# davrempe/contact-human-dynamics

Hardware: NVIDIA H100
Metric: optimised frames/sec (batched phys-optim) (higher is better)
Workload: dtype f64

## Files before the change

### contact-human-dynamics_b200/csrc/chd_api.cu

```cuda
#include <cuda_runtime.h>

#include <cstdio>
#include <cstdlib>
#include <cstring>
#include <vector>

#include "../../include/chd.h"
#include "chd_dev.h"

__global__ void chd_k_stage_begin(ChdDev D);
__global__ void chd_k_eval(ChdDev D);
__global__ void chd_k_init(ChdDev D);
__global__ void chd_k_kkt(ChdDev D);
__global__ void chd_k_kkt_gwin(ChdDev D);
__global__ void chd_k_kcopy(ChdDev D);
__global__ void chd_k_curv(ChdDev D);
__global__ void chd_k_asm(ChdDev D);
__global__ void chd_k_fp64_peak(int mode, int iters, double* sink);
__global__ void chd_k_hess_base(ChdDev D);
__global__ void chd_k_hess_dur(ChdDev D);
__global__ void chd_k_hess_zero(ChdDev D);
__global__ void chd_k_hess_fin(ChdDev D, int mode);
__global__ void chd_k_tables(ChdDev D);
__global__ void chd_k_clear_dyn(ChdDev D);
// ... 363 lines not shown
  if (b->copy_stream) cudaStreamDestroy(b->copy_stream);
  if (b->stream) cudaStreamDestroy(b->stream);
  delete b;
}

int chd_phys_get_dims(const chd_phys_batch* b, chd_phys_dims* d) {
  if (!b || !d) return -1;
  const ChdHostBatch& hb = b->hb;
  d->batch = hb.B, d->n_max = hb.n_max, d->m_max = hb.m_max, d->slots_max = hb.slots_max, d->n_splines = hb.S;
  d->p_max = hb.Pmax, d->sets_max = hb.sets_max, d->na_max = hb.Na_max, d->nb_max = hb.nb_max, d->w_max = hb.w_max;
  d->frames_out_max = hb.fo_max;
  return 0;
}
int chd_phys_get_sizes(const chd_phys_batch* b, int32_t* s) {
  if (!b || !s) return -1;
  for (int i = 0; i < b->hb.B; ++i) {
    const ChdSeq& h = b->hb.seq[i];
    s[6 * i + 0] = h.n, s[6 * i + 1] = h.m, s[6 * i + 2] = h.nslots, s[6 * i + 3] = h.Na, s[6 * i + 4] = h.nb, s[6 * i + 5] = h.w;
  }
  return 0;
}
int chd_phys_get_sizes_fixed(const chd_phys_batch* b, int32_t* s) {
  if (!b || !s) return -1;
  for (int i = 0; i < b->hb.B; ++i) s[3 * i] = b->hb.seq[i].nb_fix, s[3 * i + 1] = b->hb.seq[i].w_fix, s[3 * i + 2] = b->hb.seq[i].n_dur;
  return 0;
}
int chd_phys_get_x(const chd_phys_batch* b, double* x) {
  if (!b || !x) return -1;
  if (b->host_only) {
    std::memcpy(x, b->hb.x0.data(), b->hb.x0.size() * sizeof(double));
    return 0;
  }
  CHD_CUDA(cudaStreamSynchronize(b->stream));
  CHD_CUDA(cudaMemcpy(x, b->D.x, (size_t)b->hb.B * b->hb.n_max * sizeof(double), cudaMemcpyDeviceToHost));
  return 0;
}
int chd_phys_set_x(chd_phys_batch* b, const double* x) {
  if (!b || !x || b->host_only) return -1;
  CHD_CUDA(cudaMemcpy(b->D.x, x, (size_t)b->hb.B * b->hb.n_max * sizeof(double), cudaMemcpyHostToDevice));
  chd_k_tables<<<b->hb.B, 64, 0, b->stream>>>(b->D);
  b->launches++;
  CHD_CUDA(cudaStreamSynchronize(b->stream));
  return 0;
}

int chd_phys_eval(chd_phys_batch* b, int32_t stage, double* cost, double* grad, double* g, double* jac_vals) {
  if (!b || stage < 0 || stage > 5 || b->host_only) return -1;
  const ChdHostBatch& hb = b->hb;
  int sched[1] = {stage};
  int rc = set_schedule(b, sched, 1, -1, 0);
  if (rc) return rc;
  {
    Timer t(b, KT_INIT);
    chd_k_stage_begin<<<hb.B, CHD_THREADS, 0, b->stream>>>(b->D);
  }
  launch_eval(b);
  CHD_CUDA(cudaStreamSynchronize(b->stream));
  CHD_CUDA(cudaGetLastError());
  const size_t B = hb.B;
  if (cost) {
    std::vector<double> c2(2 * B);
    CHD_CUDA(cudaMemcpy(c2.data(), b->D.cost, 2 * B * sizeof(double), cudaMemcpyDeviceToHost));
    for (size_t i = 0; i < B; ++i) cost[i] = c2[2 * i];
  }
  if (grad) CHD_CUDA(cudaMemcpy(grad, b->D.grad, B * hb.n_max * sizeof(double), cudaMemcpyDeviceToHost));
  if (g) CHD_CUDA(cudaMemcpy(g, b->D.g, B * hb.m_max * sizeof(double), cudaMemcpyDeviceToHost));
  if (jac_vals) CHD_CUDA(cudaMemcpy(jac_vals, b->D.Jv, B * hb.slots_max * sizeof(double), cudaMemcpyDeviceToHost));
  return 0;
}

int chd_phys_get_layout(const chd_phys_batch* b, int32_t* ent_ptr, int32_t* ent_col, double* row_lo, double* row_hi,
                        int32_t* row_set, int32_t* var_kkt, int32_t* row_kkt) {
  if (!b) return -1;
  const ChdHostBatch& hb = b->hb;
  if (ent_ptr) std::memcpy(ent_ptr, hb.ent_ptr.data(), hb.ent_ptr.size() * sizeof(int));
  if (ent_col) std::memcpy(ent_col, hb.ent_col.data(), hb.ent_col.size() * sizeof(int));
  if (row_lo) std::memcpy(row_lo, hb.row_lo.data(), hb.row_lo.size() * sizeof(double));
  if (row_hi) std::memcpy(row_hi, hb.row_hi.data(), hb.row_hi.size() * sizeof(double));
  if (row_set) std::memcpy(row_set, hb.row_set.data(), hb.row_set.size() * sizeof(int));
  if (var_kkt) std::memcpy(var_kkt, hb.var_kkt.data(), hb.var_kkt.size() * sizeof(int));
  if (row_kkt) std::memcpy(row_kkt, hb.row_kkt.data(), hb.row_kkt.size() * sizeof(int));
  return 0;
}

int chd_phys_get_slot_index(const chd_phys_batch* b, int32_t* ent_row, int32_t* col_ptr, int32_t* col_ent) {
  if (!b) return -1;
  const ChdHostBatch& hb = b->hb;
  if (ent_row) std::memcpy(ent_row, hb.ent_row.data(), hb.ent_row.size() * sizeof(int));
  if (col_ptr) std::memcpy(col_ptr, hb.col_ptr.data(), hb.col_ptr.size() * sizeof(int));
  if (col_ent) std::memcpy(col_ent, hb.col_ent.data(), hb.col_ent.size() * sizeof(int));
  return 0;
}

int chd_phys_get_ent_col(const chd_phys_batch* b, int32_t* ent_col) {
  if (!b || !ent_col) return -1;
  if (b->host_only) {
    std::memcpy(ent_col, b->hb.ent_col.data(), b->hb.ent_col.size() * sizeof(int));
    return 0;
  }
  CHD_CUDA(cudaStreamSynchronize(b->stream));
  CHD_CUDA(cudaMemcpy(ent_col, b->D.ent_col, b->hb.ent_col.size() * sizeof(int), cudaMemcpyDeviceToHost));
  return 0;
}

int chd_phys_get_duals(const chd_phys_batch* b, double* y, double* zL, double* zU, double* s, double* row_scale, double* obj_scale) {
  if (!b || b->host_only) return -1;
  const size_t B = b->hb.B, mm = B * b->hb.m_max;
  CHD_CUDA(cudaStreamSynchronize(b->stream));
  if (y) CHD_CUDA(cudaMemcpy(y, b->D.y, mm * sizeof(double), cudaMemcpyDeviceToHost));
  if (zL) CHD_CUDA(cudaMemcpy(zL, b->D.zL, mm * sizeof(double), cudaMemcpyDeviceToHost));
  if (zU) CHD_CUDA(cudaMemcpy(zU, b->D.zU, mm * sizeof(double), cudaMemcpyDeviceToHost));
  if (s) CHD_CUDA(cudaMemcpy(s, b->D.s, mm * sizeof(double), cudaMemcpyDeviceToHost));
  if (row_scale) CHD_CUDA(cudaMemcpy(row_scale, b->D.sc, mm * sizeof(double), cudaMemcpyDeviceToHost));
  if (obj_scale) {
    std::vector<ChdIpm> ipm(B);
    CHD_CUDA(cudaMemcpy(ipm.data(), b->D.ipm, B * sizeof(ChdIpm), cudaMemcpyDeviceToHost));
    for (size_t i = 0; i < B; ++i) obj_scale[i] = ipm[i].sf;
  }
  return 0;
}

int chd_phys_debug_ipm(const chd_phys_batch* b, int32_t i, double* out8) {
  if (!b || !out8 || b->host_only || !b->h_ipm || i < 0 || i >= b->hb.B) return -1;
  const ChdIpm& I = b->h_ipm[i];
  out8[0] = I.a_pr, out8[1] = I.a_du, out8[2] = I.dphi, out8[3] = I.phi0, out8[4] = I.theta0, out8[5] = I.theta_ref, out8[6] = I.mu, out8[7] = I.delta_w;
  for (int q = 0; q < 8; ++q) out8[8 + q] = I.dbg[q];
  return 0;
}

int chd_phys_stage_stats(const chd_phys_batch* b, double* stats) {
  if (!b || !stats || b->host_only || !b->h_ipm) return -1;
  const int B = b->hb.B;
  for (int s = 0; s < 6; ++s)
    for (int i = 0; i < B; ++i)
      for (int q = 0; q < 4; ++q) stats[((size_t)s * B + i) * 4 + q] = b->h_ipm[i].st_stat[s][q];
  return 0;
}

int chd_phys_solve_stage(chd_phys_batch* b, int32_t stage, int32_t max_iter, int32_t* status, int32_t* iters, double* stats) {
  if (!b || stage < 0 || stage > 5 || b->host_only) return -1;
  const int B = b->hb.B;
  int sched[1] = {stage};
  int rc = set_schedule(b, sched, 1, stage, max_iter);
  if (rc) return rc;
  if ((rc = run_schedule(b))) return rc;
  for (int i = 0; i < B; ++i) {
    const ChdIpm& I = b->h_ipm[i];
    if (status) status[i] = I.st_status[stage];
    if (iters) iters[i] = I.st_iters[stage];
    if (stats) {
      double* s = stats + 8 * i;
      s[0] = I.f, s[1] = I.E0, s[2] = I.viol_u, s[3] = I.dual_u, s[4] = I.compl_u, s[5] = I.mu, s[6] = I.delta_w, s[7] = I.ls_fail;
    }
    if (i == 0 && getenv("CHD_PROF")) fprintf(stderr, "chd prof (Mcycles) seq0 stage %d: err %.2f jasm %.2f hasm %.2f factor %.2f border %.2f back %.2f rec %.2f\n", stage, I.prof[0]/1e6, I.prof[1]/1e6, I.prof[2]/1e6, I.prof[3]/1e6, I.prof[4]/1e6, I.prof[5]/1e6, I.prof[6]/1e6);
  }
  return 0;
}

int chd_phys_sample_device(chd_phys_batch* b, double* out_device, void* stream) {
  if (!b || !out_device || b->host_only) return -1;
  cudaStream_t st = stream ? (cudaStream_t)stream : b->stream;
  if (st == b->stream) {
    Timer t(b, KT_SAMPLE);
    chd_k_sample<<<b->hb.B, 128, 0, st>>>(b->D, out_device, b->d_frames);
    return 0;
  }
  cudaEvent_t ev;
  CHD_CUDA(cudaEventCreateWithFlags(&ev, cudaEventDisableTiming));
  CHD_CUDA(cudaEventRecord(ev, b->stream));
  CHD_CUDA(cudaStreamWaitEvent(st, ev, 0));
  chd_k_sample<<<b->hb.B, 128, 0, st>>>(b->D, out_device, b->d_frames);
  CHD_CUDA(cudaEventRecord(ev, st));
  CHD_CUDA(cudaStreamWaitEvent(b->stream, ev, 0));
  CHD_CUDA(cudaEventDestroy(ev));
  return 0;
}

int chd_phys_sample(chd_phys_batch* b, double* out, int32_t* frames_out) {
  if (!b || !out || b->host_only) return -1;
  const ChdHostBatch& hb = b->hb;
  const size_t stride = 6 + 7 * (size_t)hb.n_ee_max, cnt = (size_t)hb.B * hb.fo_max * stride;
  CHD_CUDA(cudaMemsetAsync(b->d_samples, 0, cnt * sizeof(double), b->stream));
  int rc = chd_phys_sample_device(b, b->d_samples, nullptr);
  if (rc) return rc;
  CHD_CUDA(cudaMemcpyAsync(out, b->d_samples, cnt * sizeof(double), cudaMemcpyDeviceToHost, b->stream));
  if (frames_out) CHD_CUDA(cudaMemcpyAsync(frames_out, b->d_frames, hb.B * sizeof(int), cudaMemcpyDeviceToHost, b->stream));
  CHD_CUDA(cudaStreamSynchronize(b->stream));
  return 0;
}

int chd_phys_solve(chd_phys_batch* b, double* samples, int32_t* frames_out, int32_t* success, int32_t* stage_status,
                   int32_t* stage_iters) {
  if (!b || b->host_only) return -1;
  const ChdHostBatch& hb = b->hb;
  const int B = hb.B;
  const size_t stride = 6 + 7 * (size_t)hb.n_ee_max, snap = (size_t)B * hb.fo_max * stride;
  int sched[6] = {CHD_STAGE_11, CHD_STAGE_12, CHD_STAGE_21, CHD_STAGE_22, CHD_STAGE_3, CHD_STAGE_4};
  int rc = set_schedule(b, sched, 6, -1, 0);
  if (rc) return rc;
  if (samples) CHD_CUDA(cudaMemsetAsync(b->D.snapshots, 0, 3 * snap * sizeof(double), b->stream));
  if ((rc = run_schedule(b))) return rc;
  for (int i = 0; i < B; ++i) {
    const ChdIpm& I = b->h_ipm[i];
    if (success) success[2 * i] = I.st_status[CHD_STAGE_22] == 0, success[2 * i + 1] = I.st_status[CHD_STAGE_3] == 0 || I.st_status[CHD_STAGE_4] == 0;
    for (int s = 0; s < 6; ++s) {
      if (stage_status) stage_status[(size_t)s * B + i] = I.st_status[s];
      if (stage_iters) stage_iters[(size_t)s * B + i] = I.st_iters[s];
    }
  }
  if (samples) CHD_CUDA(cudaMemcpyAsync(samples, b->D.snapshots, 3 * snap * sizeof(double), cudaMemcpyDeviceToHost, b->stream));
  if (frames_out) CHD_CUDA(cudaMemcpyAsync(frames_out, b->d_frames, B * sizeof(int), cudaMemcpyDeviceToHost, b->stream));
  CHD_CUDA(cudaStreamSynchronize(b->stream));
  return 0;
}

int64_t chd_phys_launch_count(const chd_phys_batch* b) { return b ? b->launches : 0; }
int64_t chd_phys_h2d_bytes(const chd_phys_batch* b) { return b ? b->h2d_bytes : 0; }
int chd_phys_reset(chd_phys_batch* b) {
  if (!b || b->host_only) return -1;
  CHD_CUDA(cudaMemcpyAsync(b->D.x, b->d_x0, (size_t)b->hb.B * b->hb.n_max * sizeof(double), cudaMemcpyDeviceToDevice, b->stream));
  const ChdHostBatch& hb = b->hb;
  CHD_CUDA(cudaMemcpyAsync(b->D.poly_T, b->poly_T0, hb.poly_T.size() * sizeof(double), cudaMemcpyDeviceToDevice, b->stream));
  CHD_CUDA(cudaMemcpyAsync(b->D.poly_tend, b->poly_tend0, hb.poly_tend.size() * sizeof(double), cudaMemcpyDeviceToDevice, b->stream));
  CHD_CUDA(cudaMemcpyAsync(b->D.phase_tend, b->phase_tend0, hb.phase_tend.size() * sizeof(double), cudaMemcpyDeviceToDevice, b->stream));
  CHD_CUDA(cudaMemcpyAsync(b->D.ent_col, b->ent_col0, hb.ent_col.size() * sizeof(int), cudaMemcpyDeviceToDevice, b->stream));
  chd_k_clear_dyn<<<(hb.B + 127) / 128, 128, 0, b->stream>>>(b->D);
  b->launches++;
  return 0;
}
int chd_phys_set_timing(chd_phys_batch* b, int enable) {
  if (!b) return -1;
  b->timing = enable;
  return 0;
}
int chd_phys_kernel_times(chd_phys_batch* b, double* ms8, int64_t* launches8, int reset) {
  if (!b) return -1;
  for (int i = 0; i < KT_N; ++i) {
    if (ms8) ms8[i] = b->kt_ms[i];
    if (launches8) launches8[i] = b->kt_n[i];
    if (reset) b->kt_ms[i] = 0, b->kt_n[i] = 0;
  }
  return 0;
}

}
```

### contact-human-dynamics_b200/csrc/chd_dev.h

```cpp
#pragma once
#include "chd_core.h"
#include "chd_layout.h"

#define CHD_FILT_MAX 24
#define CHD_THREADS 512
#define CHD_KKT_THREADS 512
#define CHD_NL_GUARD 1.0
#define CHD_NL_FLOOR 1e-4
#define CHD_UNOBS_EPS 1e-14
#define CHD_DW_UNOBS 1e-4
#define CHD_CURV_MIN 1e-8

#define CHD_ROW_ACTIVE 1
#define CHD_ROW_EQ 2
#define CHD_ROW_HASL 4
#define CHD_ROW_HASU 8
#define CHD_ROW_WARM 16

#define CHD_PH_BEGIN 0
#define CHD_PH_RUN 1
#define CHD_PH_FINISHED 2
struct ChdIpm {
  int status;
  int iter, nfilt, ls_fail, max_iter, n_bounds, m_act, pad0;
  int stage, pos, phase, snap, step_ready;
  int last_p1;
  int warm;
  int dyn;
  int band_ovf;
  int kw_req;
  int st_status[6], st_iters[6];
  double mu, delta_w, sf, theta_max, theta_min, mu_filter, tau;
  double f, E0, viol_u, dual_u, compl_u;
  double phi0, theta0, dphi, a_pr, a_du;
  double dbg[8];
  double dw_floor;
  int af_cnt, af_off;
  int af_it, af_pad;
  double af_E;
  double theta_ref;
  double filt[2 * CHD_FILT_MAX];
  double st_stat[6][4];
  double prof[8];
};

struct ChdStageDev {
  unsigned set_mask;
  int max_iter;
  int snap_after;
  int opt_dur;
  double w_data[3], w_vel[3], w_acc[3], w_dur;
};

struct ChdDev {
  int B, S, Pmax, n_max, m_max, slots_max, sets_max, tab_max, F_max, Kd_max, Kr_max, Na_max, nb_max, w_max, par_stride,
      n_ee_max, fo_max, Ph_max, win_smem, nbc_max, Q, Qfix, nbt, win_tiles, pan_doubles;
  size_t kstride;
  const ChdSeq* seq;
  double *poly_T, *poly_tend;
  const double *node_const, *par, *t_dyn, *t_rom, *t_data, *row_lo, *row_hi, *dur0;
  const int *node_var, *itab, *ent_ptr, *var_kkt, *row_kkt, *row_set, *poly_ph;
  int* ent_col;
  double *poly_Tt, *poly_tendt;
  double* jty;
  const int *ent_row, *col_ptr, *col_ent;
  const ChdSet* sets;
  double* phase_tend;
  double *x, *xt, *dx, *grad;
  double *g, *gt;
  double* Jv;
  int* rflag;
  unsigned char* unobs;
  double *sc, *dL, *dU, *s, *y, *zL, *zU, *ds, *dy, *dzL, *dzU;
  double* cost;
  double* Kwork;
  double* Kbase;
  double* sol;
  double* scratch;
  double *rhs0, *rhs1;
  size_t scratch_stride;
  ChdIpm* ipm;
  const ChdStageDev* stages;
  int sched[8], nsched;
  double* snapshots;
};

#define CHD_TOL 1e-3
#define CHD_CONSTR_VIOL_TOL 1e-4
#define CHD_DUAL_INF_TOL 1.0
#define CHD_COMPL_INF_TOL 1e-4
#define CHD_MU_INIT 0.1
#define CHD_KAPPA_EPS 10.0
#define CHD_KAPPA_MU 0.2
#define CHD_THETA_MU 1.5
#define CHD_TAU_MIN 0.99
#define CHD_KAPPA1 1e-2
#define CHD_KAPPA2 1e-2
#define CHD_KAPPA_SIGMA 1e10
#define CHD_S_MAX 100.0
#define CHD_SCAL_MAX_GRAD 100.0
#define CHD_BOUND_RELAX 1e-8
#define CHD_DELTA_W0 1e-4
#define CHD_DELTA_C 1e-8
#define CHD_DW_POLISH 1.0
#define CHD_DW_MIN 1e-8
#define CHD_AF_N 10
#define CHD_AF_MIN 1e-10
#define CHD_DW_MAX 1e4
#define CHD_DW_INC 4.0
#define CHD_DW_DEC 3.0
#define CHD_MAX_BACKTRACK 25
#define CHD_GAMMA_THETA 1e-5
#define CHD_GAMMA_PHI 1e-5
#define CHD_S_PHI 2.3
#define CHD_S_THETA 1.1
#define CHD_ETA_PHI 1e-8
#define CHD_INF 1e19

#if defined(__CUDACC__) || defined(CHD_HOST_EMU)
__device__ __forceinline__ void chd_stage_advance(const ChdDev& D, ChdIpm& I, int status, int snap_after) {
  I.st_status[I.stage] = status;
  I.st_iters[I.stage] = I.iter;
  I.st_stat[I.stage][0] = I.f, I.st_stat[I.stage][1] = I.E0, I.st_stat[I.stage][2] = I.viol_u, I.st_stat[I.stage][3] = I.dual_u;
  I.last_p1 = I.stage + 1;
  I.step_ready = 0;
  I.kw_req = 0;
  I.pos += 1;
  if (I.stage == CHD_STAGE_3 && status == 0 && I.pos < D.nsched && D.sched[I.pos] == CHD_STAGE_4) I.pos += 1;
  else if (I.stage == CHD_STAGE_3 && status != 0 && I.pos < D.nsched && D.sched[I.pos] == CHD_STAGE_4) snap_after = -1;
  I.snap = snap_after;
  if (I.pos < D.nsched) I.stage = D.sched[I.pos], I.phase = CHD_PH_BEGIN;
  else I.phase = CHD_PH_FINISHED;
}
#endif
```

### contact-human-dynamics_b200/csrc/chd_kernels.cu

```cuda
#include <cuda_runtime.h>

#include "chd_block.cuh"
#include "chd_eval.cuh"

__global__ void chd_k_stage_begin(ChdDev D) {
  const int b = blockIdx.x;
  if (D.ipm[b].phase != CHD_PH_BEGIN) return;
  const ChdStageDev sg = D.stages[D.ipm[b].stage];
  const int max_iter = sg.max_iter;
  const ChdSeq* h = D.seq + b;
  if (sg.opt_dur && h->n_dur == 0) {
    __syncthreads();
    if (threadIdx.x == 0) {
      D.ipm[b].iter = 0;
      chd_stage_advance(D, D.ipm[b], -3, sg.snap_after);
    }
    return;
  }
  const bool warm = sg.opt_dur && D.ipm[b].last_p1 == CHD_STAGE_22 + 1;
  int* rf = D.rflag + (size_t)b * D.m_max;
  const double* lo = D.row_lo + (size_t)b * D.m_max;
  const double* hi = D.row_hi + (size_t)b * D.m_max;
  const int* rset = D.row_set + (size_t)b * D.m_max;
  for (int r = threadIdx.x; r < D.m_max; r += blockDim.x) {
    int f = 0;
    if (r < h->m && (sg.set_mask & CHD_MASK(rset[r]))) {
      f = CHD_ROW_ACTIVE;
      if (lo[r] == hi[r]) f |= CHD_ROW_EQ;
      else {
        if (lo[r] > -CHD_INF) f |= CHD_ROW_HASL;
        if (hi[r] < CHD_INF) f |= CHD_ROW_HASU;
      }
      if (warm && (rf[r] & CHD_ROW_ACTIVE)) f |= CHD_ROW_WARM;
    }
    rf[r] = f;
    D.g[(size_t)b * D.m_max + r] = 0.0;
  }
  if (sg.opt_dur) {
    ChdCtx c;
    chd_make_ctx(D, b, D.x + (size_t)b * D.n_max, c);
    chd_tables_from_x(c, c.x, D.poly_T + (size_t)b * D.S * D.Pmax, D.poly_tend + (size_t)b * D.S * D.Pmax,
                      D.phase_tend + (size_t)b * D.n_ee_max * D.Ph_max);
  }
  if (threadIdx.x == 0) {
    ChdIpm& I = D.ipm[b];
    I.status = 1;
    I.iter = 0;
    I.nfilt = 0;
    I.ls_fail = 0;
    I.max_iter = max_iter;
    I.warm = warm;
    if (sg.opt_dur) I.dyn = 1;
    I.band_ovf = 0;
    if (!warm) I.mu = CHD_MU_INIT, I.sf = 1.0, I.delta_w = CHD_DELTA_W0;
    else I.delta_w = fmax(I.delta_w, CHD_DELTA_W0);
    I.mu_filter = -1.0;
    I.dw_floor = CHD_DW_MIN, I.af_cnt = 0, I.af_off = 0, I.af_it = 0, I.af_E = 0.0;
    for (int q = 0; q < 8; ++q) I.prof[q] = 0.0;
    for (int q = 40; q < 48; ++q) I.filt[q] = 0.0;
  }
}

__global__ void __launch_bounds__(CHD_THREADS) chd_k_eval(ChdDev D) {
  extern __shared__ double sm[];
  const int b = blockIdx.x;
  if (D.ipm[b].phase != CHD_PH_BEGIN && D.ipm[b].phase != CHD_PH_RUN) return;
  const ChdStageDev sg = D.stages[D.ipm[b].stage];
  const ChdSeq* h = D.seq + b;
  double* xs = sm;
  double* gs = sm + D.n_max;
  double* red = sm + 2 * D.n_max;
  const double* x = D.x + (size_t)b * D.n_max;
  for (int i = threadIdx.x; i < h->n; i += blockDim.x) xs[i] = x[i], gs[i] = 0.0;
  __syncthreads();
  ChdCtx c;
  chd_make_ctx(D, b, xs, c);
  c.dyn = D.ipm[b].dyn;
  c.opt_dur = sg.opt_dur;
  chd_eval_all<true>(c, sg, D.g + (size_t)b * D.m_max, D.Jv + (size_t)b * D.slots_max, gs, D.cost + 2 * b, red);
  double* grad = D.grad + (size_t)b * D.n_max;
  for (int i = threadIdx.x; i < h->n; i += blockDim.x) grad[i] = gs[i];
}

__global__ void __launch_bounds__(CHD_THREADS) chd_k_init(ChdDev D) {
  __shared__ double red[CHD_THREADS];
  const int b = blockIdx.x;
  if (D.ipm[b].phase != CHD_PH_BEGIN) return;
  const ChdSeq* h = D.seq + b;
  const size_t ro = (size_t)b * D.m_max;
  const int* vk = D.var_kkt + (size_t)b * D.n_max;
  const double* grad = D.grad + (size_t)b * D.n_max;
  double gm = 0.0;
  for (int i = threadIdx.x; i < h->n; i += blockDim.x)
    if (vk[i] >= 0) gm = fmax(gm, fabs(grad[i]));
  gm = chd_block_max(gm, red);
  const bool warm = D.ipm[b].warm;
  const double mu0 = D.ipm[b].mu;
  const double sf = warm ? D.ipm[b].sf : (gm > CHD_SCAL_MAX_GRAD ? CHD_SCAL_MAX_GRAD / gm : 1.0);
  const int* ep = D.ent_ptr + (size_t)b * (D.m_max + 1);
  const int* ec = D.ent_col + (size_t)b * D.slots_max;
  const double* Jv = D.Jv + (size_t)b * D.slots_max;
  int nb_l = 0;
  for (int r = threadIdx.x; r < h->m; r += blockDim.x) {
    const int f = D.rflag[ro + r];
    if (!(f & CHD_ROW_ACTIVE)) continue;
    if (f & CHD_ROW_WARM) {
      if (!(f & CHD_ROW_EQ)) nb_l += ((f & CHD_ROW_HASL) ? 1 : 0) + ((f & CHD_ROW_HASU) ? 1 : 0);
      continue;
    }
    double rm = 0.0;
    for (int e = ep[r]; e < ep[r + 1]; ++e) {
      const int col = ec[e];
      if (col >= 0 && vk[col] >= 0) rm = fmax(rm, fabs(Jv[e]));
    }
    double sc = rm > CHD_SCAL_MAX_GRAD ? CHD_SCAL_MAX_GRAD / rm : 1.0;
    sc = fmax(sc, 1e-8);
    D.sc[ro + r] = sc;
    const double lo = D.row_lo[ro + r] * sc, hi = D.row_hi[ro + r] * sc;
    const double d = sc * D.g[ro + r];
    D.y[ro + r] = 0.0;
    if (f & CHD_ROW_EQ) {
      D.dL[ro + r] = lo, D.dU[ro + r] = hi, D.s[ro + r] = d, D.zL[ro + r] = 0.0, D.zU[ro + r] = 0.0;
      continue;
    }
    const bool hl = f & CHD_ROW_HASL, hu = f & CHD_ROW_HASU;
    const double dL = hl ? lo - CHD_BOUND_RELAX * fmax(1.0, fabs(lo)) : -INFINITY;
    const double dU = hu ? hi + CHD_BOUND_RELAX * fmax(1.0, fabs(hi)) : INFINITY;
    double s = d;
    if (hl) {
      double pL = CHD_KAPPA1 * fmax(1.0, fabs(dL));
      if (hu) pL = fmin(pL, CHD_KAPPA2 * (dU - dL));
      s = fmax(s, dL + pL);
    }
    if (hu) {
      double pU = CHD_KAPPA1 * fmax(1.0, fabs(dU));
      if (hl) pU = fmin(pU, CHD_KAPPA2 * (dU - dL));
      s = fmin(s, dU - pU);
    }
    D.dL[ro + r] = dL, D.dU[ro + r] = dU, D.s[ro + r] = s;
    D.zL[ro + r] = hl ? (warm ? mu0 / (s - dL) : 1.0) : 0.0;
    D.zU[ro + r] = hu ? (warm ? mu0 / (dU - s) : 1.0) : 0.0;
    nb_l += (hl ? 1 : 0) + (hu ? 1 : 0);
  }
  const double nbnd = chd_block_sum((double)nb_l, red);
  int act = 0;
  for (int r = threadIdx.x; r < h->m; r += blockDim.x) act += (D.rflag[ro + r] & CHD_ROW_ACTIVE) ? 1 : 0;
  const double nact = chd_block_sum((double)act, red);
  if (threadIdx.x == 0) {
    D.ipm[b].sf = sf;
    D.ipm[b].n_bounds = (int)nbnd;
    D.ipm[b].m_act = (int)nact;
  }
}

__global__ void __launch_bounds__(CHD_THREADS) chd_k_linesearch(ChdDev D) {
  extern __shared__ double sm[];
  __shared__ int s_ok, s_ftype, s_trust;
  __shared__ double s_cost;
  const int b = blockIdx.x;
  ChdIpm& I = D.ipm[b];
  if (I.phase != CHD_PH_RUN || !I.step_ready) return;
  const ChdStageDev sg = D.stages[I.stage];
  const ChdSeq* h = D.seq + b;
  const int n = h->n, m = h->m, tid = threadIdx.x, nt = blockDim.x;
  const size_t ro = (size_t)b * D.m_max, vo = (size_t)b * D.n_max;
  const int* rf = D.rflag + ro;
  double* xt = sm;
  double* red = sm + D.n_max;
  const double* x = D.x + vo;
  const double* dx = D.dx + vo;
  double* gt = D.gt + ro;
  const double mu = I.mu, sf = I.sf, theta = I.theta0, phi0 = I.phi0, dphi = I.dphi, a_pr = I.a_pr, a_du = I.a_du;
  if (a_pr == 0.0 && dphi == 0.0) {
    if (tid == 0) I.iter += 1, I.step_ready = 0;
    return;
  }
  ChdCtx c;
  chd_make_ctx(D, b, xt, c);
  c.dyn = I.dyn;
  c.opt_dur = sg.opt_dur;
  if (sg.opt_dur) {
    c.poly_T = D.poly_Tt + (size_t)b * D.S * D.Pmax;
    c.poly_tend = D.poly_tendt + (size_t)b * D.S * D.Pmax;
    const size_t cnt = (size_t)D.S * D.Pmax;
    for (size_t i = tid; i < cnt; i += nt) {
      D.poly_Tt[(size_t)b * cnt + i] = D.poly_T[(size_t)b * cnt + i];
      D.poly_tendt[(size_t)b * cnt + i] = D.poly_tend[(size_t)b * cnt + i];
    }
    __syncthreads();
  }
  const double theta_ref = I.theta_ref;
  double alpha = a_pr;
  int ls = 0;
  bool accepted = false, ftype = false;
  for (ls = 0; ls < CHD_MAX_BACKTRACK; ++ls) {
    for (int i = tid; i < n; i += nt) xt[i] = x[i] + alpha * dx[i];
    __syncthreads();
    if (sg.opt_dur) {
      if (tid == 0) s_trust = 0;
      __syncthreads();
      if (tid < h->n_ee) {
        double t = 0.0, t0 = 0.0;
        int bad = 0;
        for (int k = 0; k < h->n_phases[tid] - 1; ++k) {
          t += xt[h->dur_xoff[tid] + k];
          t0 += c.dur0[(size_t)tid * c.Ph_max + k];
          if (fabs(t - t0) > CHD_TAU_TRUST) bad = 1;
        }
        if (bad) s_trust = 1;
      }
      chd_tables_from_x(c, xt, D.poly_Tt + (size_t)b * D.S * D.Pmax, D.poly_tendt + (size_t)b * D.S * D.Pmax, nullptr);
// ... 186 lines not shown
```

### contact-human-dynamics_b200/csrc/chd_kkt.cu

```cuda
#include <cuda_runtime.h>

#include "chd_block.cuh"
#include "chd_eval.cuh"
#include "chd_kkt_tiles.cuh"

__device__ __forceinline__ void chd_hess_sample(const ChdCtx& c, const ChdKT& K, const int* vk, int s, const ChdSpl* P, const double* sign, int np,
                                                int deriv, double wgt, int lane, double* ws) {
  const bool tau = c.opt_dur && s >= 2 && deriv == 0;
  if (lane < 28) {
    const int pa = lane / 14, q = lane % 14;
    double v0 = 0.0, v1 = 0.0, v2 = 0.0;
    int ia = -1;
    if (pa < np) {
      if (q < 12) {
        const int va = P[pa].var[q];
        const double wa = sign[pa] * chd_slot_w(P[pa], deriv, q);
        if (va >= 0 && wa != 0.0) {
          ia = vk[va];
          v0 = q % 3 == 0 ? wa : 0.0, v1 = q % 3 == 1 ? wa : 0.0, v2 = q % 3 == 2 ? wa : 0.0;
        }
      } else if (tau) {
        ChdTau u;
        chd_spl_tau(c, s, s - 2, P[pa], u);
        const int var = q == 12 ? u.va : u.vb;
// ... 515 lines not shown
  int na;
  {
    const int g1 = lane + 32;
    const bool act0 = lane < Gm && (lane >= GB || lane < tq) && gnz[lane];
    const bool act1 = g1 < Gm && (g1 >= GB || g1 < tq) && gnz[g1 < 96 ? g1 : 0];
    const unsigned m0 = __ballot_sync(0xffffffffu, act0), m1 = __ballot_sync(0xffffffffu, act1);
    const unsigned below = (1u << lane) - 1u;
    const int n0 = __popc(m0);
    na = n0 + __popc(m1);
    if (act0) cmp[__popc(m0 & below)] = (unsigned char)lane;
    if (act1) cmp[n0 + __popc(m1 & below)] = (unsigned char)g1;
    __syncwarp();
  }
  auto corner = [&](const double* X, const double* Y, int bi, int bj) {
    double* Cc = c.cc + (size_t)(bi * 8 + (lane >> 2)) * nbp8 + bj * 8 + 2 * (lane & 3);
    double c0 = Cc[0], c1 = Cc[1];
    chd_tile_mma(c0, c1, X, Y, lane);
    Cc[0] = c0, Cc[1] = c1;
  };
  const int step = c.nwarp - 1, r8 = (lane >> 2) * 8 + 2 * (lane & 3);
  const int nb2 = (na + 1) >> 1, nblk = nb2 * (nb2 + 1) / 2;
  for (int p = warp - 1; p < nblk; p += step) {
    const int bi = s_pairs[p] >> 8, bj = s_pairs[p] & 255;
    const int i1 = 2 * bi + 1, j1 = 2 * bj + 1;
    const bool vi1 = i1 < na, vj1 = j1 < na;
    int gi[2], gj[2];
    gi[0] = cmp[2 * bi], gi[1] = cmp[i1 & 63];
    gj[0] = cmp[2 * bj], gj[1] = cmp[j1 & 63];
    double2 xf[2], yf[2];
    xf[0] = *reinterpret_cast<const double2*>(xpan + gi[0] * 64 + 2 * lane);
    yf[0] = *reinterpret_cast<const double2*>(ypan + gj[0] * 64 + 2 * lane);
    xf[1] = vi1 ? *reinterpret_cast<const double2*>(xpan + gi[1] * 64 + 2 * lane) : make_double2(0.0, 0.0);
    yf[1] = vj1 ? *reinterpret_cast<const double2*>(ypan + gj[1] * 64 + 2 * lane) : make_double2(0.0, 0.0);
    double* Cp[4];
    double2 cv[4];
#pragma unroll
    for (int t = 0; t < 4; ++t) {
      const int a = t & 1, cl = t >> 1;
      bool ok = (a == 0 || vi1) && (cl == 0 || vj1) && !(bi == bj && a == 0 && cl == 1);
      const int g_i = gi[a], g_j = gj[cl];
      ok = ok && !(g_i == 0 && g_j == 0);
      Cp[t] = nullptr;
      if (ok) {
        if (g_i < GB) Cp[t] = band_tile(g_i, g_j);
        else if (g_j < GB) Cp[t] = bord_tile(g_i - GB, g_j);
        else corner(xpan + g_i * 64, ypan + g_j * 64, g_i - GB, g_j - GB);
      }
      if (Cp[t]) cv[t] = *reinterpret_cast<const double2*>(Cp[t] + r8);
    }
#pragma unroll
    for (int t = 0; t < 4; ++t)
      if (Cp[t]) {
        const double2 xa = xf[t & 1], yb = yf[t >> 1];
        asm volatile("mma.sync.aligned.m8n8k4.row.col.f64.f64.f64.f64 {%0,%1}, {%2}, {%3}, {%0,%1};"
                     : "+d"(cv[t].x), "+d"(cv[t].y)
                     : "d"(-xa.x), "d"(yb.x));
      }
#pragma unroll
    for (int t = 0; t < 4; ++t)
      if (Cp[t]) {
        const double2 xa = xf[t & 1], yb = yf[t >> 1];
        asm volatile("mma.sync.aligned.m8n8k4.row.col.f64.f64.f64.f64 {%0,%1}, {%2}, {%3}, {%0,%1};"
                     : "+d"(cv[t].x), "+d"(cv[t].y)
                     : "d"(-xa.y), "d"(yb.y));
        *reinterpret_cast<double2*>(Cp[t] + r8) = cv[t];
      }
  }
}

template <class BandTile, class BordTile>
__device__ __forceinline__ void chd_kkt_update_wide(const ChdKktCtx& c, const unsigned short* s_pairs, const int* gnz, int GB, int npairs,
                                                    int tq, const BandTile& band_tile, const BordTile& bord_tile) {
  const int lane = c.lane, nwarp = c.nwarp, nbp8 = c.nbp8;
  const double *xpan = c.xpan, *ypan = c.ypan;
  double* cc = c.cc;
  const int r8 = (lane >> 2) * 8 + 2 * (lane & 3);
  int p = c.warp - 1;
  while (p < npairs) {
    struct { double* C; const double *X, *Y; } tl[4];
    int nq = 0;
    while (nq < 4 && p < npairs) {
      const int gi = s_pairs[p] >> 8, gj = s_pairs[p] & 255;
      p += nwarp - 1;
      if ((gi < GB && gi >= tq) || (gj < GB && gj >= tq) || !gnz[gi] || !gnz[gj]) continue;
      if (gi == 0 && gj == 0) continue;
      const double* X = xpan + gi * 64;
      const double* Y = ypan + gj * 64;
      if (gi < GB) {
        tl[nq].C = band_tile(gi, gj), tl[nq].X = X, tl[nq].Y = Y, ++nq;
      } else if (gj < GB) {
        tl[nq].C = bord_tile(gi - GB, gj), tl[nq].X = X, tl[nq].Y = Y, ++nq;
      } else {
        const int bi = gi - GB, bj = gj - GB;
        for (int e = lane; e < 64; e += 32) {
          const int r = e >> 3, cq = e & 7;
          double acc = 0.0;
#pragma unroll
          for (int kk = 0; kk < 8; ++kk) acc += X[r * 8 + kk] * Y[cq * 8 + kk];
          cc[(bi * 8 + r) * nbp8 + bj * 8 + cq] -= acc;
        }
      }
    }
    double c0[4], c1[4];
#pragma unroll
    for (int i = 0; i < 4; ++i)
      if (i < nq) c0[i] = tl[i].C[r8], c1[i] = tl[i].C[r8 + 1];
#pragma unroll
    for (int i = 0; i < 4; ++i)
      if (i < nq) {
        chd_tile_mma(c0[i], c1[i], tl[i].X, tl[i].Y, lane);
        tl[i].C[r8] = c0[i], tl[i].C[r8 + 1] = c1[i];
      }
  }
}

template <bool WS>
__device__ __forceinline__ void chd_kkt_factor(const ChdKktCtx& c, int& s_fail) {
  const ChdKT& K = c.K;
  const int tid = c.tid, nt = c.nt, lane = c.lane, warp = c.warp, nwarp = c.nwarp;
  const int Qs = c.Qs, Q = c.Q, nbt = c.nbt, nbp8 = c.nbp8, nbc = c.nbc, nbt_s = c.nbt_s;
  double *cc = c.cc, *ypan = c.ypan, *xpan = c.xpan, *dinv = c.dinv, *win = c.win, *bwin = c.bwin;
  for (int i = tid; i < nbp8 * nbp8; i += nt) cc[i] = K.corn[i];
  if (WS) {
    for (int idx = tid; idx < Q * Q * 64; idx += nt) {
      const int e = idx & 63, pr = idx >> 6, J = pr / Q, t = pr % Q;
      if (J + t < Q && J < nbc && J + t < nbc) win[chd_win_slot(J + t, J, Q) * 64 + e] = K.band[((size_t)J * Qs + t) * 64 + e];
    }
    for (int idx = tid; idx < Q * nbt * 64; idx += nt) {
      const int J = idx / (nbt * 64);
      if (J < nbc) bwin[idx] = K.bord[(size_t)J * nbt * 64 + idx % (nbt * 64)];
    }
  }
  __syncthreads();
  __shared__ int s_rs[2][96];
  __shared__ int s_gnz[2][96];
  __shared__ unsigned short s_pairs[3000];
  __shared__ unsigned char s_cmp[CHD_KKT_THREADS / 32][64];
  __shared__ __align__(16) double s_winv[2][64];
  const int GB = K.q, Gm = K.q + nbt_s, npairs = Gm * (Gm + 1) / 2;
  for (int p = tid; p < npairs && p < 3000; p += nt) {
    int gi = (int)((sqrt(8.0 * p + 1.0) - 1.0) * 0.5);
    while (gi * (gi + 1) / 2 > p) --gi;
    while ((gi + 1) * (gi + 2) / 2 <= p) ++gi;
    s_pairs[p] = (unsigned short)((gi << 8) | (p - gi * (gi + 1) / 2));
  }
  auto tri = [](int a_, int b_) { return a_ > b_ ? a_ * (a_ + 1) / 2 + b_ : b_ * (b_ + 1) / 2 + a_; };
  for (int g = tid; g < GB; g += nt) s_rs[0][g] = (1 + g) % Q;
  for (int g = tid; g < 96; g += nt) s_gnz[0][g] = 0, s_gnz[1][g] = 0;
  if (warp == 0) {
    const bool ok = chd_tile_ldl(WS ? win : K.band, dinv, s_winv[0], lane);
    if (!ok && lane == 0) s_fail = 1;
  }
  __syncthreads();
  int kslot = 0, cur = 0;
  for (int Kc = 0; Kc < nbc; ++Kc, cur ^= 1) {
    const int tq = min(K.q, nbc - 1 - Kc);
    const int* rs = s_rs[cur];
    auto band_tile = [&](int gi, int gj) -> double* {
      return WS ? win + (size_t)tri(rs[gi], rs[gj]) * 64 : K.band + ((size_t)(Kc + 1 + gj) * Qs + (gi - gj)) * 64;
    };
    auto bord_tile = [&](int bi, int gj) -> double* {
      return WS ? bwin + ((size_t)rs[gj] * nbt + bi) * 64 : K.bord + ((size_t)(Kc + 1 + gj) * nbt + bi) * 64;
    };
    double* Tkk = WS ? win + (size_t)tri(kslot, kslot) * 64 : K.band + (size_t)Kc * Qs * 64;
    double* Bk = WS ? bwin + (size_t)kslot * nbt * 64 : K.bord + (size_t)Kc * nbt * 64;
    const double* dv = dinv + 8 * cur;
    {
      const double* wv = s_winv[cur];
      const int r = lane >> 2, k = lane & 3;
      const double2 wf = *reinterpret_cast<const double2*>(wv + 2 * lane);
      const double d0 = dv[2 * k], d1 = dv[2 * k + 1];
      const int f0 = r * 8 + chd_frag_col(2 * k), f1 = r * 8 + chd_frag_col(2 * k + 1);
      for (int g = warp; g < tq + nbt_s; g += nwarp) {
        const bool band_t = g < tq;
        const int pg = band_t ? g : GB + (g - tq);
        const double* A = band_t ? (WS ? win + (size_t)tri(rs[g], kslot) * 64 : K.band + ((size_t)Kc * Qs + 1 + g) * 64) : Bk + (g - tq) * 64;
        const double ax = A[r * 8 + k], ay = A[r * 8 + k + 4];
        double c0 = 0.0, c1 = 0.0;
        asm volatile("mma.sync.aligned.m8n8k4.row.col.f64.f64.f64.f64 {%0,%1}, {%2}, {%3}, {%0,%1};"
                     : "+d"(c0), "+d"(c1)
                     : "d"(ax), "d"(wf.x));
        asm volatile("mma.sync.aligned.m8n8k4.row.col.f64.f64.f64.f64 {%0,%1}, {%2}, {%3}, {%0,%1};"
                     : "+d"(c0), "+d"(c1)
                     : "d"(ay), "d"(wf.y));
        const double x0 = c0 * d0, x1 = c1 * d1;
        ypan[pg * 64 + f0] = c0, ypan[pg * 64 + f1] = c1;
        xpan[pg * 64 + f0] = x0, xpan[pg * 64 + f1] = x1;
        double* G = band_t ? K.band + ((size_t)Kc * Qs + 1 + g) * 64 : K.bord + ((size_t)Kc * nbt + (g - tq)) * 64;
        *reinterpret_cast<double2*>(G + r * 8 + 2 * k) = make_double2(x0, x1);
        const bool nz = __any_sync(0xffffffffu, x0 != 0.0 || x1 != 0.0);
        if (lane == 0 && nz) s_gnz[cur][pg] = 1;
      }
    }
    if (WS)
      for (int e = tid; e < 64; e += nt) K.band[(size_t)Kc * Qs * 64 + e] = Tkk[e];
    __syncthreads();
    const int In = Kc + Q;
    if (WS && In < nbc) {
      for (int idx = tid - 32; idx < Q * 32 + nbt_s * 32; idx += nt - 32) {
        if (idx < 0) break;
        const int tile = idx >> 5, off = (idx & 31) * 2;
        if (tile < Q) {
          const int J = tile < GB ? Kc + 1 + tile : In;
          double* dst = tile < GB ? win + (size_t)tri(kslot, rs[tile]) * 64 : Tkk;
          chd_copy16(dst + off, K.band + ((size_t)J * Qs + (In - J)) * 64 + off, WS);
        } else {
          chd_copy16(Bk + (tile - Q) * 64 + off, K.bord + (size_t)In * nbt * 64 + (tile - Q) * 64 + off, WS);
        }
      }
    }
    if (warp == 0) {
      if (tq >= 1) {
        double* Tn = band_tile(0, 0);
        chd_tile_sub_xyT(Tn, xpan, ypan, lane);
        __syncwarp();
        const bool ok = chd_tile_ldl(Tn, dinv + 8 * (cur ^ 1), s_winv[cur ^ 1], lane);
        if (!ok && lane == 0) s_fail = 1;
      }
    } else {
      if (warp == 1) {
        for (int g = lane; g < GB; g += 32) {
          int v = kslot + 2 + g;
          while (v >= Q) v -= Q;
          s_rs[cur ^ 1][g] = v;
        }
        for (int g = lane; g < Gm; g += 32) s_gnz[cur ^ 1][g] = 0;
      }
      if (!WS && Gm > 64) chd_kkt_update_wide(c, s_pairs, s_gnz[cur], GB, npairs, tq, band_tile, bord_tile);
      else chd_kkt_update_compact(c, s_pairs, s_cmp[warp], s_gnz[cur], GB, Gm, tq, band_tile, bord_tile);
    }
    chd_copy_wait(WS);
    __syncthreads();
    kslot = kslot + 1 == Q ? 0 : kslot + 1;
  }
}

__device__ __forceinline__ void chd_kkt_border(const ChdDev& D, const ChdKktCtx& c, int& s_fail) {
  const int tid = c.tid, nt = c.nt, lane = c.lane, warp = c.warp, nbl = c.nbl, nbp8 = c.nbp8, NBR = c.NBR, Na = c.K.Na;
  double* cc = c.cc;
  for (int k = 0; k < nbl; ++k) {
    const double dk = cc[k * nbp8 + k];
    if (tid == 0 && !(dk > 0.0 && isfinite(dk))) s_fail = 1;
    __syncthreads();
    const double ik = 1.0 / dk;
    const int rem = nbl - k - 1;
    for (int idx = tid; idx < rem * rem; idx += nt) {
      const int i = k + 1 + idx / rem, j = k + 1 + idx % rem;
      if (j <= i) cc[i * nbp8 + j] -= cc[i * nbp8 + k] * ik * cc[j * nbp8 + k];
    }
    for (int j = k + 1 + tid; j < nbl; j += nt) cc[NBR * nbp8 + j] -= cc[j * nbp8 + k] * ik * cc[NBR * nbp8 + k];
    __syncthreads();
  }
  double* xb = c.xs + 8 * D.nbc_max;
  if (warp == 0) {
    for (int j = lane; j < nbl; j += 32) xb[j] = cc[NBR * nbp8 + j];
    __syncwarp();
    for (int k = nbl - 1; k >= 0; --k) {
      const double xk = xb[k] / cc[k * nbp8 + k];
      __syncwarp();
      for (int j = lane; j < k; j += 32) xb[j] -= cc[k * nbp8 + j] * xk;
      if (lane == 0) xb[k] = xk;
      __syncwarp();
    }
  }
  __syncthreads();
  for (int i = tid; i < nbl; i += nt) D.sol[(size_t)c.b * (D.Na_max + D.nb_max) + Na + i] = xb[i];
}

template <bool WS>
__device__ __forceinline__ void chd_kkt_backsub(const ChdDev& D, const ChdKktCtx& c) {
  const ChdKT& K = c.K;
  const int tid = c.tid, nt = c.nt, lane = c.lane, warp = c.warp, Q = c.Q, Qs = c.Qs, nbt = c.nbt, nbl = c.nbl, nbc = c.nbc;
  const int NBR = c.NBR, Na = K.Na;
  double *xs = c.xs, *sol = D.sol + (size_t)c.b * (D.Na_max + D.nb_max);
  const double* xb = xs + 8 * D.nbc_max;
  double* accv = c.xs2;
  for (int i = tid; i < K.Np; i += nt) {
    const double* bt = K.bord + (size_t)(i >> 3) * nbt * 64 + (i & 7);
    double v = bt[NBR * 8];
    for (int q2 = 0; q2 < nbl; ++q2) v -= bt[q2 * 8] * xb[q2];
    accv[i] = v;
  }
  const int per = Q * 64;
  const int R = max(1, (int)((c.win_region - (WS ? c.n_even + c.xs_len : 0)) / 64) / (2 * Q));
  double* stg = c.win;
  auto stage_chunk = [&](int Ktop, int buf, int t0, int tstep) {
    for (int idx = t0; idx < R * Q * 32; idx += tstep) {
      const int rr = idx / (Q * 32), rem = idx - rr * (Q * 32);
      const int Kr = Ktop - rr;
      if (Kr < 0) break;
      const int tile = rem >> 5, off = (rem & 31) * 2;
      const int J = tile == 0 ? Kr : Kr - tile;
      if (J < 0) continue;
      chd_copy16(stg + ((size_t)buf * R + rr) * per + tile * 64 + off, K.band + ((size_t)J * Qs + (Kr - J)) * 64 + off, WS);
    }
  };
  stage_chunk(nbc - 1, 0, tid, nt);
  chd_copy_wait(WS);
  __syncthreads();
  int buf = 0;
  for (int Ktop = nbc - 1; Ktop >= 0; Ktop -= R, buf ^= 1) {
    if (warp != 0) {
      stage_chunk(Ktop - R, buf ^ 1, tid - 32, nt - 32);
    } else {
      for (int rr = 0; rr < R && Ktop - rr >= 0; ++rr) {
        const int Kc = Ktop - rr;
        const double* T0 = stg + ((size_t)buf * R + rr) * per;
        double xk[8];
#pragma unroll
        for (int cl = 7; cl >= 0; --cl) {
          double v = accv[Kc * 8 + cl];
#pragma unroll
          for (int p = 7; p > cl; --p) v -= T0[p * 8 + cl] * xk[p];
          xk[cl] = v;
        }
        if (lane < 8) {
          const int gi = Kc * 8 + lane;
          double v = xk[0];
#pragma unroll
          for (int cl = 1; cl < 8; ++cl) v = lane == cl ? xk[cl] : v;
          xs[gi] = v;
          if (gi < Na) sol[gi] = v;
        }
        const int nrow = min(K.q, Kc);
        for (int idx = lane; idx < nrow * 8; idx += 32) {
          const int g = idx >> 3, cl = idx & 7;
          const double* T = T0 + (g + 1) * 64;
          double v = 0.0;
#pragma unroll
          for (int r = 0; r < 8; ++r) v += T[r * 8 + cl] * xk[r];
          accv[(Kc - 1 - g) * 8 + cl] -= v;
        }
        __syncwarp();
      }
    }
    chd_copy_wait(WS);
    __syncthreads();
  }
}

__device__ __forceinline__ bool chd_kkt_no_step(const ChdDev& D, const ChdKktCtx& c, const int& s_fail) {
  ChdIpm& I = *c.I;
  const int tid = c.tid, nt = c.nt, n = c.n, m = c.m;
  const size_t ro = c.ro, vo = c.vo;
  if (I.band_ovf) {
    __syncthreads();
    if (tid == 0) I.status = -2, chd_stage_advance(D, I, -2, c.sg.snap_after);
    return true;
  }
  if (s_fail) {
    if (tid == 0) {
      I.delta_w = fmin(fmax(I.delta_w * 100.0, 1e-4), CHD_DW_MAX * 10);
      I.a_pr = 0.0, I.a_du = 0.0, I.dphi = 0.0;
      I.ls_fail += 1;
      I.step_ready = 1;
      I.kw_req = 1;
      if (I.delta_w > CHD_DW_MAX) I.status = -2, chd_stage_advance(D, I, -2, c.sg.snap_after);
    }
    for (int i = tid; i < n; i += nt) D.dx[vo + i] = 0.0;
    for (int r = tid; r < m; r += nt) D.ds[ro + r] = 0.0, D.dy[ro + r] = 0.0, D.dzL[ro + r] = 0.0, D.dzU[ro + r] = 0.0;
    return true;
  }
  return false;
}

__device__ __forceinline__ void chd_kkt_recover(const ChdDev& D, const ChdKktCtx& c) {
  ChdIpm& I = *c.I;
  const ChdSeq* h = c.h;
  const int b = c.b, tid = c.tid, nt = c.nt, n = c.n, m = c.m, n_act = c.n_act;
  const size_t ro = c.ro, vo = c.vo;
  const int *rf = c.rf, *vk = c.vk, *rk = c.rk, *ep = c.ep, *ec = c.ec;
  const double *Jv = c.Jv, *grad = c.grad, *sol = D.sol + (size_t)c.b * (D.Na_max + D.nb_max), sf = c.sf, mu = c.mu, tau = c.tau;
  double *vecn = c.vecn, *red = c.red;
  double* dx = D.dx + vo;
  for (int i = tid; i < n; i += nt) {
    const int k = vk[i];
    const double v = (k >= 0 && i < n_act) ? sol[k] : 0.0;
    dx[i] = v;
    vecn[i] = v;
  }
  __syncthreads();
  if (c.sg.opt_dur) {
    for (int ee = 0; ee < h->n_ee; ++ee)
      for (int k = 1 + tid; k < h->n_phases[ee] - 1; k += nt) dx[h->dur_xoff[ee] + k] = vecn[h->dur_xoff[ee] + k] - vecn[h->dur_xoff[ee] + k - 1];
  }
  double a_pr = 1.0, a_du = 1.0, a_dphi = 0.0, a_phi = 0.0;
  for (int i = tid; i < n; i += nt) a_dphi += sf * grad[i] * vecn[i];
  for (int r = tid; r < m; r += nt) {
    const int f = rf[r];
    if (!(f & CHD_ROW_ACTIVE)) continue;
    if (f & CHD_ROW_EQ) {
      D.dy[ro + r] = sol[rk[r]];
      D.ds[ro + r] = 0.0;
      continue;
    }
    const double sc = D.sc[ro + r], s = D.s[ro + r];
    double Jdx = 0.0;
    for (int e = ep[r]; e < ep[r + 1]; ++e) {
      const int col = ec[e];
      if (col >= 0) Jdx += Jv[e] * vecn[col];
    }
    const double riq = sc * D.g[ro + r] - s;
    const double ds = sc * Jdx + riq;
    const bool hl = f & CHD_ROW_HASL, hu = f & CHD_ROW_HASU;
    const double gapL = hl ? s - D.dL[ro + r] : 1.0, gapU = hu ? D.dU[ro + r] - s : 1.0;
    const double zL = D.zL[ro + r], zU = D.zU[ro + r];
    const double sigL = hl ? zL / gapL : 0.0, sigU = hu ? zU / gapU : 0.0;
    const double bvec = (hl ? mu / gapL : 0.0) - (hu ? mu / gapU : 0.0);
    const double dy = (sigL + sigU) * ds - D.y[ro + r] - bvec;
    const double dzL = hl ? mu / gapL - zL - sigL * ds : 0.0;
    const double dzU = hu ? mu / gapU - zU + sigU * ds : 0.0;
    D.ds[ro + r] = ds, D.dy[ro + r] = dy, D.dzL[ro + r] = dzL, D.dzU[ro + r] = dzU;
    if (hl && ds < 0) a_pr = fmin(a_pr, -tau * gapL / ds);
    if (hu && ds > 0) a_pr = fmin(a_pr, tau * gapU / ds);
    if (hl && dzL < 0) a_du = fmin(a_du, -tau * zL / dzL);
    if (hu && dzU < 0) a_du = fmin(a_du, -tau * zU / dzU);
    if (hl) a_dphi -= mu * ds / gapL, a_phi -= mu * log(gapL);
    if (hu) a_dphi += mu * ds / gapU, a_phi -= mu * log(gapU);
  }
  a_pr = chd_block_min(a_pr, red);
  a_du = chd_block_min(a_du, red);
  const double dphi = chd_block_sum(a_dphi, red);
  const double phib = chd_block_sum(a_phi, red);
  if (tid == 0) {
    I.a_pr = a_pr, I.a_du = a_du, I.dphi = dphi;
    I.phi0 = sf * D.cost[2 * b] + phib;
    I.step_ready = 1;
    I.kw_req = 1;
  }
}

template <bool WS>
__device__ __forceinline__ void chd_kkt_body(const ChdDev& D) {
  __shared__ int s_fail;
  ChdIpm& I = D.ipm[blockIdx.x];
  if (I.phase != CHD_PH_RUN) return;
  ChdKktCtx c;
  chd_kkt_ctx_init<WS>(D, I, c);
#ifdef CHD_PROFILE
  long long tk0 = clock64();
#define CHD_PROF(slot) do { __syncthreads(); if (c.tid == 0) { long long t_ = clock64(); I.prof[slot] += (double)(t_ - tk0); tk0 = t_; } } while (0)
#else
#define CHD_PROF(slot) do { } while (0)
#endif
  if (chd_kkt_errors(D, c, s_fail)) return;
  CHD_PROF(0);
  chd_kkt_assemble(D, c);
  CHD_PROF(1);
  if (!c.pre_refreshed) chd_curv_rows(D, c.b, c.K, c.sg, c.warp, c.nwarp, c.lane, c.win + c.warp * 192);
  __threadfence_block();
  __syncthreads();
  CHD_PROF(2);
  chd_kkt_factor<WS>(c, s_fail);
  CHD_PROF(3);
  chd_kkt_border(D, c, s_fail);
  CHD_PROF(4);
  chd_kkt_backsub<WS>(D, c);
  CHD_PROF(5);
  if (chd_kkt_no_step(D, c, s_fail)) return;
  __syncthreads();
  chd_kkt_recover(D, c);
  CHD_PROF(6);
}
#undef CHD_PROF

__global__ void __launch_bounds__(256) chd_k_kcopy(ChdDev D) {
  const int b = blockIdx.y;
  if (!D.ipm[b].kw_req) return;
  if (blockIdx.x == 0) {
    const size_t go = (size_t)b * (D.Na_max + D.nb_max);
    for (int i = threadIdx.x; i < D.Na_max + D.nb_max; i += blockDim.x) D.rhs0[go + i] = 0.0, D.rhs1[go + i] = 0.0;
  }
  if (D.stages[D.ipm[b].stage].opt_dur && D.ipm[b].phase == CHD_PH_RUN) {
    chd_hess_clear(D, b, D.Kwork + (size_t)b * D.kstride, blockIdx.x, gridDim.x);
    return;
  }
  const size_t cnt2 = D.kstride / 2, per = (cnt2 + gridDim.x - 1) / gridDim.x;
  const size_t lo = (size_t)blockIdx.x * per, hi = lo + per < cnt2 ? lo + per : cnt2;
  chd_kwork_copy(D, b, lo + threadIdx.x, hi, blockDim.x);
}

__global__ void __launch_bounds__(256) chd_k_curv(ChdDev D) {
  __shared__ double s_ws[8 * 192];
  const int b = blockIdx.y;
  const ChdIpm& I = D.ipm[b];
  if (!I.kw_req || I.phase != CHD_PH_RUN) return;
// ... 47 lines not shown
```

Before: 11900.

## Split banded back-substitution across three warps with named barrier handoff

```diff
diff --git a/contact-human-dynamics_b200/csrc/chd_api.cu b/contact-human-dynamics_b200/csrc/chd_api.cu
--- a/contact-human-dynamics_b200/csrc/chd_api.cu
+++ b/contact-human-dynamics_b200/csrc/chd_api.cu
@@ -539,7 +539,12 @@
       double* s = stats + 8 * i;
       s[0] = I.f, s[1] = I.E0, s[2] = I.viol_u, s[3] = I.dual_u, s[4] = I.compl_u, s[5] = I.mu, s[6] = I.delta_w, s[7] = I.ls_fail;
     }
-    if (i == 0 && getenv("CHD_PROF")) fprintf(stderr, "chd prof (Mcycles) seq0 stage %d: err %.2f jasm %.2f hasm %.2f factor %.2f border %.2f back %.2f rec %.2f\n", stage, I.prof[0]/1e6, I.prof[1]/1e6, I.prof[2]/1e6, I.prof[3]/1e6, I.prof[4]/1e6, I.prof[5]/1e6, I.prof[6]/1e6);
+    if (i == 0 && getenv("CHD_PROF")) {
+      fprintf(stderr, "chd prof (Mcycles) seq0 stage %d: err %.2f jasm %.2f hasm %.2f factor %.2f border %.2f back %.2f rec %.2f\n", stage, I.prof[0]/1e6, I.prof[1]/1e6, I.prof[2]/1e6, I.prof[3]/1e6, I.prof[4]/1e6, I.prof[5]/1e6, I.prof[6]/1e6);
+      const double ncol = I.prof[10] > 0 ? I.prof[10] : 1.0;
+      fprintf(stderr, "chd prof (cycles per block column, %.0f columns) seq0 stage %d: diag tile %.0f update+stream-in %.0f panel %.0f whole column %.0f\n",
+              I.prof[10], stage, I.prof[7] / ncol, I.prof[8] / ncol, I.prof[9] / ncol, I.prof[3] / ncol);
+    }
   }
   return 0;
 }
diff --git a/contact-human-dynamics_b200/csrc/chd_dev.h b/contact-human-dynamics_b200/csrc/chd_dev.h
--- a/contact-human-dynamics_b200/csrc/chd_dev.h
+++ b/contact-human-dynamics_b200/csrc/chd_dev.h
@@ -41,7 +41,7 @@
   double theta_ref;
   double filt[2 * CHD_FILT_MAX];
   double st_stat[6][4];
-  double prof[8];
+  double prof[12];
 };
 
 struct ChdStageDev {
diff --git a/contact-human-dynamics_b200/csrc/chd_kernels.cu b/contact-human-dynamics_b200/csrc/chd_kernels.cu
--- a/contact-human-dynamics_b200/csrc/chd_kernels.cu
+++ b/contact-human-dynamics_b200/csrc/chd_kernels.cu
@@ -56,7 +56,7 @@
     else I.delta_w = fmax(I.delta_w, CHD_DELTA_W0);
     I.mu_filter = -1.0;
     I.dw_floor = CHD_DW_MIN, I.af_cnt = 0, I.af_off = 0, I.af_it = 0, I.af_E = 0.0;
-    for (int q = 0; q < 8; ++q) I.prof[q] = 0.0;
+    for (int q = 0; q < 12; ++q) I.prof[q] = 0.0;
     for (int q = 40; q < 48; ++q) I.filt[q] = 0.0;
   }
 }
diff --git a/contact-human-dynamics_b200/csrc/chd_kkt.cu b/contact-human-dynamics_b200/csrc/chd_kkt.cu
--- a/contact-human-dynamics_b200/csrc/chd_kkt.cu
+++ b/contact-human-dynamics_b200/csrc/chd_kkt.cu
@@ -691,8 +691,18 @@
     if (!ok && lane == 0) s_fail = 1;
   }
   __syncthreads();
+#ifdef CHD_PROFILE
+  __shared__ unsigned long long s_pu;
+  long long p_pan = 0, p_diag = 0, p_upd = 0;
+  if (tid == 0) s_pu = 0;
+  __syncthreads();
+#define CHD_PROF_T(v) long long v = clock64()
+#else
+#define CHD_PROF_T(v) do { } while (0)
+#endif
   int kslot = 0, cur = 0;
   for (int Kc = 0; Kc < nbc; ++Kc, cur ^= 1) {
+    CHD_PROF_T(t_col);
     const int tq = min(K.q, nbc - 1 - Kc);
     const int* rs = s_rs[cur];
     auto band_tile = [&](int gi, int gj) -> double* {
@@ -734,6 +744,10 @@
     if (WS)
       for (int e = tid; e < 64; e += nt) K.band[(size_t)Kc * Qs * 64 + e] = Tkk[e];
     __syncthreads();
+    CHD_PROF_T(t_upd);
+#ifdef CHD_PROFILE
+    p_pan += t_upd - t_col;
+#endif
     const int In = Kc + Q;
     if (WS && In < nbc) {
       for (int idx = tid - 32; idx < Q * 32 + nbt_s * 32; idx += nt - 32) {
@@ -756,6 +770,9 @@
         const bool ok = chd_tile_ldl(Tn, dinv + 8 * (cur ^ 1), s_winv[cur ^ 1], lane);
         if (!ok && lane == 0) s_fail = 1;
       }
+#ifdef CHD_PROFILE
+      p_diag += clock64() - t_upd;
+#endif
     } else {
       if (warp == 1) {
         for (int g = lane; g < GB; g += 32) {
@@ -769,9 +786,19 @@
       else chd_kkt_update_compact(c, s_pairs, s_cmp[warp], s_gnz[cur], GB, Gm, tq, band_tile, bord_tile);
     }
     chd_copy_wait(WS);
+#ifdef CHD_PROFILE
+    if (warp > 0 && lane == 0) atomicMax(&s_pu, (unsigned long long)(clock64() - t_upd));
+#endif
     __syncthreads();
+#ifdef CHD_PROFILE
+    if (tid == 0) p_upd += (long long)s_pu, s_pu = 0;
+#endif
     kslot = kslot + 1 == Q ? 0 : kslot + 1;
   }
+#ifdef CHD_PROFILE
+  if (tid == 0) c.I->prof[7] += (double)p_diag, c.I->prof[8] += (double)p_upd, c.I->prof[9] += (double)p_pan, c.I->prof[10] += (double)nbc;
+#endif
+#undef CHD_PROF_T
 }
 
 __device__ __forceinline__ void chd_kkt_border(const ChdDev& D, const ChdKktCtx& c, int& s_fail) {
@@ -837,40 +864,51 @@
   stage_chunk(nbc - 1, 0, tid, nt);
   chd_copy_wait(WS);
   __syncthreads();
+  double* xkb = c.dinv;
+  auto row_update = [&](const double* T0, const double* xk, int Kc, int g, int cl) {
+    const double* T = T0 + (g + 1) * 64;
+    double v = 0.0;
+#pragma unroll
+    for (int r = 0; r < 8; ++r) v += T[r * 8 + cl] * xk[r];
+    accv[(Kc - 1 - g) * 8 + cl] -= v;
+  };
   int buf = 0;
   for (int Ktop = nbc - 1; Ktop >= 0; Ktop -= R, buf ^= 1) {
-    if (warp != 0) {
-      stage_chunk(Ktop - R, buf ^ 1, tid - 32, nt - 32);
+    if (warp > 2) {
+      stage_chunk(Ktop - R, buf ^ 1, tid - 96, nt - 96);
     } else {
       for (int rr = 0; rr < R && Ktop - rr >= 0; ++rr) {
         const int Kc = Ktop - rr;
         const double* T0 = stg + ((size_t)buf * R + rr) * per;
+        const int nrow = min(K.q, Kc);
         double xk[8];
-#pragma unroll
-        for (int cl = 7; cl >= 0; --cl) {
-          double v = accv[Kc * 8 + cl];
-#pragma unroll
-          for (int p = 7; p > cl; --p) v -= T0[p * 8 + cl] * xk[p];
-          xk[cl] = v;
+        if (warp == 0) {
+#pragma unroll
+          for (int cl = 7; cl >= 0; --cl) {
+            double v = accv[Kc * 8 + cl];
+#pragma unroll
+            for (int p = 7; p > cl; --p) v -= T0[p * 8 + cl] * xk[p];
+            xk[cl] = v;
+          }
+          if (lane < 8) {
+            const int gi = Kc * 8 + lane;
+            double v = xk[0];
+#pragma unroll
+            for (int cl = 1; cl < 8; ++cl) v = lane == cl ? xk[cl] : v;
+            xs[gi] = v;
+            if (gi < Na) sol[gi] = v;
+            xkb[(Kc & 1) * 8 + lane] = v;
+          }
         }
-        if (lane < 8) {
-          const int gi = Kc * 8 + lane;
-          double v = xk[0];
-#pragma unroll
-          for (int cl = 1; cl < 8; ++cl) v = lane == cl ? xk[cl] : v;
-          xs[gi] = v;
-          if (gi < Na) sol[gi] = v;
+        asm volatile("bar.sync 1, 96;" ::: "memory");
+        if (warp == 0) {
+          if (lane < 8 && nrow > 0) row_update(T0, xk, Kc, 0, lane);
+          __syncwarp();
+        } else {
+#pragma unroll
+          for (int r = 0; r < 8; ++r) xk[r] = xkb[(Kc & 1) * 8 + r];
+          for (int idx = 8 + (warp - 1) * 32 + lane; idx < nrow * 8; idx += 64) row_update(T0, xk, Kc, idx >> 3, idx & 7);
         }
-        const int nrow = min(K.q, Kc);
-        for (int idx = lane; idx < nrow * 8; idx += 32) {
-          const int g = idx >> 3, cl = idx & 7;
-          const double* T = T0 + (g + 1) * 64;
-          double v = 0.0;
-#pragma unroll
-          for (int r = 0; r < 8; ++r) v += T[r * 8 + cl] * xk[r];
-          accv[(Kc - 1 - g) * 8 + cl] -= v;
-        }
-        __syncwarp();
       }
     }
     chd_copy_wait(WS);
```

Measured after the change: 12540, median of 6. 5.4% higher.
